# NSAPH-Projects/weather2alert

Hardware: AMD Instinct MI355X
Metric: env_steps_per_sec (higher is better)
Workload: dtype f32 tables, fp64 logit accumulation, f32 sigmoid/reward

## Files before the change

weather2alert_amd/csrc/w2a_step64.hip.h:

```cpp
#ifndef W2A_STEP64_HIP_H
#define W2A_STEP64_HIP_H

#ifndef W2A_S64_MIN_ENVS
#define W2A_S64_MIN_ENVS 131072
#endif
#define S64_ENVS 64
#define S64_WAVES (BLOCK / 64)
#define S64_PASS_ENVS 32
#define S64_ROUNDS 4

struct Day {
  uint32_t t, used, streak, hist, ndays, atb, actual, used2, hist2, st_bits, last;
  int32_t budget, act;
  bool done;
};
__device__ __forceinline__ Day derive_day(const u3 h, const u3 c, int32_t act) {
  Day d;
  d.st_bits = 0;
  if (act != 0 && act != 1) { d.st_bits |= W2A_ST_BAD_ACTION; act = 1; }
  d.act = act;
  d.last = D0_LAST(h.a);
  d.t = D0_T(h.a); d.used = D0_USED(h.a); d.streak = D0_STREAK(h.a);
  d.hist = D1_HIST(h.b); d.ndays = D1_NDAYS(h.b);
  d.budget = (int32_t)c.a;
  if (D1_FIN(h.b)) d.st_bits |= W2A_ST_STEP_AFTER_DONE;
  d.atb = ((int32_t)d.used == d.budget) ? 1u : 0u;
  d.actual = (act == 1 && d.atb) ? 0u : (uint32_t)act;
  d.used2 = d.used + d.actual;
  d.hist2 = ((d.hist << 1) | d.actual) & 0x3FFFu;
  d.done = (d.t + 1 >= d.ndays);
  return d;
}
__device__ __forceinline__ float4 runtime_fields(const Day &d, bool fix_lag = false) {
  return make_float4((d.t > 0) ? (float)(fix_lag ? d.last : d.actual) : 0.0f, (float)d.streak,
                     (float)(d.budget - (int32_t)d.used2), (float)__popc(d.hist2));
}
__device__ __forceinline__ void set_comp4(float4 &x, int idx, float v) {
  if (idx == 0) x.x = v;
  if (idx == 1) x.y = v;
  if (idx == 2) x.z = v;
  if (idx == 3) x.w = v;
}

template <bool FIXES>
struct S64WaveT {
  uint2 desc[S64_ENVS];
  float4 rt[S64_ENVS];
  float4 rt2[FIXES ? S64_ENVS : 1];
  float2 z[S64_ENVS];
  float tile[S64_PASS_ENVS * ROWF];
};

#ifndef W2A_S64_SC1
#define W2A_S64_SC1 0
#endif
#ifndef W2A_S64_SKIP_EFF
#define W2A_S64_SKIP_EFF 1
#endif
#ifndef W2A_S64_NT_STATE
#define W2A_S64_NT_STATE 0
#endif
typedef uint32_t v3u __attribute__((ext_vector_type(3)));
__device__ __forceinline__ void st16_sc1(void *p, v4f v) {
  asm volatile("global_store_dwordx4 %0, %1, off sc1" ::"v"(p), "v"(v) : "memory");
}
__device__ __forceinline__ void st12_sc1(void *p, v3u v) {
  asm volatile("global_store_dwordx3 %0, %1, off sc1" ::"v"(p), "v"(v) : "memory");
}
typedef uint32_t v2u __attribute__((ext_vector_type(2)));
__device__ __forceinline__ void st8_sc1(void *p, v2u v) {
  asm volatile("global_store_dwordx2 %0, %1, off sc1" ::"v"(p), "v"(v) : "memory");
}
__device__ __forceinline__ void st4_sc1(void *p, uint32_t v) {
  asm volatile("global_store_dword %0, %1, off sc1" ::"v"(p), "v"(v) : "memory");
}
__device__ __forceinline__ void st1_sc1(void *p, uint32_t v) {
  asm volatile("global_store_byte %0, %1, off sc1" ::"v"(p), "v"(v) : "memory");
}

#ifndef W2A_S64_MIN_WAVES
#define W2A_S64_MIN_WAVES 4
#endif
#ifndef W2A_S64_PRIO
#define W2A_S64_PRIO 3
#endif
#ifndef W2A_S64_TILES
#define W2A_S64_TILES 1
#endif
#ifndef W2A_S64_SERPENTINE
#define W2A_S64_SERPENTINE 1
#endif
__device__ __forceinline__ uint32_t logical_block_rev(uint32_t b, uint32_t per_xcd) {
#if W2A_XCD_SWIZZLE
  return (b & 7u) * per_xcd + (per_xcd - 1u - (b >> 3));
#else
  return 8u * per_xcd - 1u - b;
#endif
}
template <bool WRITE_OBS, bool REWARD_GIVEN, bool PACKED, bool AUTORESET = false, bool FIXES = false>
__device__ __forceinline__ void s64_tile(const StepArgs &a, S64WaveT<FIXES> &sw, const int lane, const int64_t wave_env0,
                                         const bool valid, const uint32_t e, const u3 h, const u3 c, const int32_t act,
                                         const int4 so) {
  const Day d = derive_day(h, c, act);
  const uint32_t t = d.t, used2 = d.used2, hist2 = d.hist2, streak = d.streak, ndays = d.ndays;
  const uint32_t actual = d.actual, atb = d.atb, st_bits = d.st_bits;
  const int32_t budget = d.budget;
  const bool done = d.done;
  const bool restart_in = AUTORESET && a.next_step && D1_FIN(h.b);
  const uint32_t fx = FIXES ? a.tb.fixes : 0u;
  const bool fix_obs = FIXES && WRITE_OBS && (fx & W2A_FIX_OBS);
  uint32_t need_eff = actual;
  if (a.tb.gate_bits && actual)
    need_eff = (a.tb.gate_bits[t * (uint32_t)a.tb.gate_words + (c.b >> 5)] >> (c.b & 31u)) & 1u;
  {
    const uint32_t day_row = t * (uint32_t)(a.tb.S_w * a.tb.Y) + c.b;
    const uint32_t wrow = W_COL(c.c) * (uint32_t)a.tb.n_samples + W_SAMPLE(c.c);
    sw.desc[lane] = make_uint2((day_row * (ROWF / 4)) | ((fix_obs && !done) ? 0x80000000u : 0u),
                               (wrow * (2 * ROWF / 4)) | (need_eff << 31));
    sw.rt[lane] = runtime_fields(d, (fx & W2A_FIX_LAG) != 0u);
    if (fix_obs)
      sw.rt2[FIXES ? lane : 0] = make_float4((float)actual, (float)(actual ? streak + 1 : 0), (float)(budget - (int32_t)used2),
                                 (float)__popc(hist2));
  }
  __builtin_amdgcn_fence(__ATOMIC_RELEASE, "wavefront");
  __builtin_amdgcn_wave_barrier();
  __builtin_amdgcn_fence(__ATOMIC_ACQUIRE, "wavefront");

  const int p = lane & 7;
  const int g = lane >> 3;
  const int n_obs = a.tb.n_obs;
  const bool write_me = valid && (!done || fix_obs) && !restart_in;
  const uint32_t next_day = (uint32_t)(a.tb.S_w * a.tb.Y) * (ROWF / 4);
#pragma unroll 1
  for (int pass = 0; pass < S64_ENVS / S64_PASS_ENVS; ++pass) {
    if (REWARD_GIVEN && !WRITE_OBS) break;
    if (wave_env0 + pass * S64_PASS_ENVS >= a.n) break;
    float4 x[S64_ROUNDS], wb[S64_ROUNDS], we[S64_ROUNDS], xo[FIXES ? S64_ROUNDS : 1];
    bool need[S64_ROUNDS], nxt[S64_ROUNDS];
#pragma unroll
    for (int r = 0; r < S64_ROUNDS; ++r) {
      uint2 ds = sw.desc[pass * S64_PASS_ENVS + r * 8 + g];
      need[r] = (ds.y >> 31) != 0u;
      nxt[r] = FIXES && (ds.x >> 31) != 0u;
      if (FIXES) ds.x &= 0x7FFFFFFFu;
      const uint32_t wq = ds.y & 0x7FFFFFFFu;
      x[r] = a.tb.X[ds.x + p];
      if (fix_obs) xo[r] = a.tb.X[ds.x + (nxt[r] ? next_day : 0u) + p];
      wb[r] = we[r] = make_float4(0.f, 0.f, 0.f, 0.f);
      if (!REWARD_GIVEN) {
        wb[r] = a.tb.W[wq + p];
        we[r] = a.tb.W[wq + (need[r] ? ROWF / 4 : 0) + p];
      }
    }
#if W2A_S64_PRIO
    __builtin_amdgcn_s_setprio(W2A_S64_PRIO);
#endif
#pragma unroll
    for (int r = 0; r < S64_ROUNDS; ++r) {
      const int j = pass * S64_PASS_ENVS + r * 8 + g;
      if (p == RT_QUAD) x[r] = sw.rt[j];
      if (FIXES && (fx & W2A_FIX_ALERTS_2WKS) && a.tb.slot_hist2w >= 0) {
        const float a2w = sw.rt[j].w;
        if (p == (a.tb.slot_hist2w >> 2)) set_comp4(x[r], a.tb.slot_hist2w & 3, a2w);
        if (fix_obs && p == (a.tb.slot_hist2w >> 2)) set_comp4(xo[r], a.tb.slot_hist2w & 3, a2w);
      }
      if (fix_obs && p == RT_QUAD) xo[r] = nxt[r] ? sw.rt2[FIXES ? j : 0] : sw.rt[j];
      if (!REWARD_GIVEN) {
      const double x0 = (double)x[r].x, x1 = (double)x[r].y, x2 = (double)x[r].z, x3 = (double)x[r].w;
      double zb = x0 * (double)wb[r].x;
      zb = fma(x1, (double)wb[r].y, zb);
      zb = fma(x2, (double)wb[r].z, zb);
      zb = fma(x3, (double)wb[r].w, zb);
      zb += dpp_f64<0xB1>(zb);
      zb += dpp_f64<0x4E>(zb);
      zb += dpp_f64<0x141>(zb);
      double ze = 0.0;
#if W2A_S64_SKIP_EFF
      if (__any(need[r]))
#endif
      {
        ze = x0 * (double)we[r].x;
        ze = fma(x1, (double)we[r].y, ze);
        ze = fma(x2, (double)we[r].z, ze);
        ze = fma(x3, (double)we[r].w, ze);
        if (p == GATE_QUAD && !(x[r].z > 0.5f)) ze = -__builtin_inf();
        ze += dpp_f64<0xB1>(ze);
        ze += dpp_f64<0x4E>(ze);
        ze += dpp_f64<0x141>(ze);
      }
      if (p == 0) sw.z[j] = make_float2((float)zb, (float)ze);
      }
      if (WRITE_OBS) {
        const int base = (r * 8 + g) * n_obs;
        const int trash = S64_PASS_ENVS * n_obs + (lane & 31);
        const float4 ov = fix_obs ? xo[FIXES ? r : 0] : x[r];
        sw.tile[so.x >= 0 ? base + so.x : trash] = ov.x;
        sw.tile[so.y >= 0 ? base + so.y : trash] = ov.y;
        sw.tile[so.z >= 0 ? base + so.z : trash] = ov.z;
        sw.tile[so.w >= 0 ? base + so.w : trash] = ov.w;
      }
    }
    if (WRITE_OBS) {
      __builtin_amdgcn_fence(__ATOMIC_RELEASE, "wavefront");
      __builtin_amdgcn_wave_barrier();
      __builtin_amdgcn_fence(__ATOMIC_ACQUIRE, "wavefront");
      const int64_t env0 = wave_env0 + pass * S64_PASS_ENVS;
      float *dst = reinterpret_cast<float *>(a.obs) + env0 * n_obs;
      const unsigned long long wm_all = __ballot(write_me);
      const uint32_t wm = (uint32_t)(wm_all >> (pass * S64_PASS_ENVS));
      const bool full = env0 + S64_PASS_ENVS <= a.n;
      if (full && wm == 0xFFFFFFFFu) {
        const int chunks = (S64_PASS_ENVS * n_obs) >> 2;
#pragma unroll
        for (int c0 = 0; c0 < (S64_PASS_ENVS * ROWF) / 4; c0 += 64) {
          const int ch = c0 + lane;
          if (ch < chunks) {
            const v4f v = reinterpret_cast<const v4f *>(sw.tile)[ch];
#if W2A_S64_SC1 & 1
            st16_sc1(reinterpret_cast<v4f *>(dst) + ch, v);
#elif W2A_NT_OBS
            __builtin_nontemporal_store(v, reinterpret_cast<v4f *>(dst) + ch);
#else
            reinterpret_cast<v4f *>(dst)[ch] = v;
#endif
          }
        }
      } else if (wm != 0u) {
        const int total = S64_PASS_ENVS * n_obs;
        for (int i = lane; i < total; i += 64) {
          const int jj = i / n_obs;
          if ((wm >> jj) & 1u) dst[i] = sw.tile[i];
        }
      }
      __builtin_amdgcn_fence(__ATOMIC_RELEASE, "wavefront");
      __builtin_amdgcn_wave_barrier();
      __builtin_amdgcn_fence(__ATOMIC_ACQUIRE, "wavefront");
    }
  }
  if (!WRITE_OBS) {
    __builtin_amdgcn_fence(__ATOMIC_RELEASE, "wavefront");
    __builtin_amdgcn_wave_barrier();
    __builtin_amdgcn_fence(__ATOMIC_ACQUIRE, "wavefront");
  }

#if W2A_S64_PRIO
  __builtin_amdgcn_s_setprio(0);
#endif
  if (AUTORESET && valid && restart_in) {
    a.reward[e] = 0.0f;
    a.done[e] = 0;
  } else if (valid && a.skip_finished && D1_FIN(h.b)) {
    a.reward[e] = 0.0f;
    a.done[e] = 1;
  } else if (valid) {
  float r;
  if (REWARD_GIVEN) {
    r = a.reward[e];
  } else {
    const float2 z = sw.z[lane];
    const float base = sigmoid_f32(z.x);
    const float eff = need_eff ? sigmoid_f32(z.y) : 0.0f;
    r = -(1000.0f / 152.0f) * base * (1.0f - eff);
    if (FIXES && (fx & W2A_FIX_PENALTY) && d.act == 1 && atb) r = -1.0f;
  }
  const uint32_t t2 = done ? t : t + 1;
  const uint32_t streak2 = done ? streak : (actual ? streak + 1 : 0);
  const float ret = __uint_as_float(h.c) + r;
  u3 h2;
  h2.a = pack_d0(t2, used2, streak2, actual, atb);
  h2.b = pack_d1(hist2, ndays, done ? 1u : 0u);
  h2.c = __float_as_uint(ret);
#if W2A_S64_SC1 & 2
  if (PACKED) st8_sc1(&a.st.pk_hot[e], v2u{pk_pack_hot(used2, streak2, hist2, done ? 1u : 0u), h2.c});
  else st12_sc1(&a.st.hot3[e], v3u{h2.a, h2.b, h2.c});
  if (!REWARD_GIVEN) st4_sc1(&a.reward[e], __float_as_uint(r));
  st1_sc1(&a.done[e], done ? 1u : 0u);
#else
  if (PACKED) a.st.pk_hot[e] = make_uint2(pk_pack_hot(used2, streak2, hist2, done ? 1u : 0u), h2.c);
  else a.st.hot3[e] = h2;
  if (!REWARD_GIVEN) a.reward[e] = r;
  a.done[e] = done ? 1 : 0;
#endif
  if (PACKED && lane == 0) a.st.pk_day[wave_env0 >> 6] = t2;
  if (done && a.last_return) a.last_return[e] = ret;
  if (st_bits) atomicOr(a.status, (int)st_bits);
  }
  if (AUTORESET) {
    const bool rs = valid && (a.next_step ? restart_in : done);
    const unsigned long long rs_mask = __ballot(rs);
    if (rs_mask) {
      uint2 ds = make_uint2(0xFFFFFFFFu, 0u);
      if (rs) {
        const uint4 cold = load_cold(a.st, e);
        const Episode ep = draw_episode(a.tb, a.rc, (uint64_t)(a.gid0 + e), cold.w + 1, (int32_t)cold.z);
        if (ep.bad) atomicOr(a.status, (int)W2A_ST_BAD_EPISODE);
        store_episode(a.st, e, make_uint4(ep.ep_row, ep.ep_w, (uint32_t)ep.sticky, cold.w + 1),
                      make_uint4(pack_d0(0, 0, 0, 0, 0), pack_d1(0, ep.ndays, 0), __float_as_uint(0.0f), (uint32_t)ep.budget));
        if (PACKED) {
          a.st.pk_hot[e] = make_uint2(pk_pack_hot(0u, 0u, 0u, 0u), __float_as_uint(0.0f));
          a.st.pk_c[e] = make_uint2(pk_budget16((uint32_t)ep.budget) | (W_COL(ep.ep_w) << 16),
                                    (ep.ep_row & 0x3FFFFFu) | (W_SAMPLE(ep.ep_w) << 22));
        }
        ds = make_uint2(ep.ep_row * (ROWF / 4), (uint32_t)ep.budget);
      }
      if (WRITE_OBS) {
        sw.desc[lane] = ds;
        __builtin_amdgcn_fence(__ATOMIC_RELEASE, "wavefront");
        __builtin_amdgcn_wave_barrier();
        __builtin_amdgcn_fence(__ATOMIC_ACQUIRE, "wavefront");
#pragma unroll 1
        for (int r = 0; r < S64_ENVS / 8; ++r) {
          if (!((rs_mask >> (r * 8)) & 0xFFull)) continue;
          const int j = r * 8 + g;
          const uint2 dj = sw.desc[j];
          if (dj.x != 0xFFFFFFFFu) {
            float4 v = a.tb.X[dj.x + p];
            if (p == RT_QUAD) v = make_float4(0.0f, 0.0f, (float)(int32_t)dj.y, 0.0f);
            if (FIXES && (fx & W2A_FIX_ALERTS_2WKS) && a.tb.slot_hist2w >= 0 && p == (a.tb.slot_hist2w >> 2))
              set_comp4(v, a.tb.slot_hist2w & 3, 0.0f);
            float *row = reinterpret_cast<float *>(a.obs) + (size_t)(wave_env0 + j) * n_obs;
            if (so.x >= 0) row[so.x] = v.x;
            if (so.y >= 0) row[so.y] = v.y;
            if (so.z >= 0) row[so.z] = v.z;
            if (so.w >= 0) row[so.w] = v.w;
          }
        }
      }
      if (PACKED && lane == 0) a.st.pk_day[wave_env0 >> 6] = 0u;
    }
  }
}

__device__ __forceinline__ void s64_load_packed(const StepArgs &a, uint32_t e, uint32_t day, u3 &h, u3 &c, int32_t &act) {
#if W2A_S64_NT_STATE & 4
  const v2u phv = __builtin_nontemporal_load(reinterpret_cast<const v2u *>(&a.st.pk_hot[e]));
  const v2u pcv = __builtin_nontemporal_load(reinterpret_cast<const v2u *>(&a.st.pk_c[e]));
  const uint2 ph = make_uint2(phv.x, phv.y), pc = make_uint2(pcv.x, pcv.y);
#else
  const uint2 ph = a.st.pk_hot[e];
  const uint2 pc = a.st.pk_c[e];
#endif
  h.a = pack_d0(day, PK_USED(ph.x), PK_STREAK(ph.x), PK_HIST(ph.x) & 1u, 0u);
  h.b = pack_d1(PK_HIST(ph.x), (uint32_t)a.uni_nd, PK_FIN(ph.x));
  h.c = ph.y;
  c.a = pc.x & 0xFFFFu;
  if (c.a == PK_BUDGET_ESCAPE) c.a = a.st.stepc[e].a;
  c.b = pc.y & 0x3FFFFFu;
  c.c = PACK_W(pc.x >> 16, pc.y >> 22);
  act = load_action(a, e);
}
__device__ __forceinline__ void s64_load_state(const StepArgs &a, uint32_t e, u3 &h, u3 &c, int32_t &act) {
#if W2A_S64_NT_STATE & 1
  const v3u hv = __builtin_nontemporal_load(reinterpret_cast<const v3u *>(&a.st.hot3[e]));
  h.a = hv.x; h.b = hv.y; h.c = hv.z;
#else
  h = a.st.hot3[e];
#endif
#if W2A_S64_NT_STATE & 2
  const v3u cv = __builtin_nontemporal_load(reinterpret_cast<const v3u *>(&a.st.stepc[e]));
  c.a = cv.x; c.b = cv.y; c.c = cv.z;
#else
  c = a.st.stepc[e];
#endif
  act = load_action(a, e);
}

template <bool WRITE_OBS, bool REWARD_GIVEN, bool PACKED = false, bool AUTORESET = false, bool FIXES = false>
__global__ __launch_bounds__(BLOCK, FIXES ? 3 : W2A_S64_MIN_WAVES) void k_step64(const StepArgs a) {
  __shared__ __attribute__((aligned(16))) S64WaveT<FIXES> s_w[S64_WAVES];
  const int tid = threadIdx.x;
  const int lane = tid & 63;
  const int wave = __builtin_amdgcn_readfirstlane(tid >> 6);
  S64WaveT<FIXES> &sw = s_w[wave];
  uint32_t lb = logical_block(blockIdx.x, gridDim.x >> 3);
  int wave_tile = wave;
#if W2A_S64_SERPENTINE
  if (a.walk_rev) {
    lb = logical_block_rev(blockIdx.x, gridDim.x >> 3);
    wave_tile = S64_WAVES - 1 - wave;
  }
#endif
  const int64_t wave_env0 = ((int64_t)lb * S64_WAVES + wave_tile) * (S64_ENVS * W2A_S64_TILES);
  if (wave_env0 >= a.n) return;
  uint32_t dayn = 0;
  if (PACKED) {
    dayn = a.st.pk_day[wave_env0 >> 6];
    if (dayn == W2A_PK_DAY_POISON) {
      if (lane == 0) atomicOr(a.status, (int)W2A_ST_STALE_GRAPH);
      return;
    }
  }
  u3 hn, cn;
  int32_t an;
  {
    const int64_t env = wave_env0 + lane;
    if (PACKED) s64_load_packed(a, (uint32_t)(env < a.n ? env : a.n - 1), dayn, hn, cn, an);
    else s64_load_state(a, (uint32_t)(env < a.n ? env : a.n - 1), hn, cn, an);
  }
  int4 so = make_int4(-1, -1, -1, -1);
  if (WRITE_OBS) so = reinterpret_cast<const int4 *>(a.slot_obs)[lane & 7];
#pragma unroll 1
  for (int i = 0; i < W2A_S64_TILES; ++i) {
    const int64_t env0 = wave_env0 + (int64_t)i * S64_ENVS;
    if (env0 >= a.n) break;
    const int64_t env = env0 + lane;
    const bool valid = env < a.n;
    const uint32_t e = (uint32_t)(valid ? env : (a.n - 1));
    const u3 h = hn, c = cn;
    const int32_t act = an;
    if (i + 1 < W2A_S64_TILES && env0 + S64_ENVS < a.n) {
      const int64_t en = env + S64_ENVS;
      if (PACKED) {
        dayn = a.st.pk_day[(env0 + S64_ENVS) >> 6];
        s64_load_packed(a, (uint32_t)(en < a.n ? en : a.n - 1), dayn == W2A_PK_DAY_POISON ? 0u : dayn, hn, cn, an);
      } else s64_load_state(a, (uint32_t)(en < a.n ? en : a.n - 1), hn, cn, an);
    }
    s64_tile<WRITE_OBS, REWARD_GIVEN, PACKED, AUTORESET, FIXES>(a, sw, lane, env0, valid, e, h, c, act, so);
    __builtin_amdgcn_fence(__ATOMIC_RELEASE, "wavefront");
    __builtin_amdgcn_wave_barrier();
    __builtin_amdgcn_fence(__ATOMIC_ACQUIRE, "wavefront");
  }
}

__global__ void k_pack_state(StateArrays st, int64_t n) {
  const int64_t i = (int64_t)blockIdx.x * blockDim.x + threadIdx.x;
  if (i >= n) return;
  const u3 h = st.hot3[i];
  const u3 c = st.stepc[i];
  st.pk_hot[i] = make_uint2(pk_pack_hot(D0_USED(h.a), D0_STREAK(h.a), D1_HIST(h.b), D1_FIN(h.b)), h.c);
  st.pk_c[i] = make_uint2(pk_budget16(c.a) | (W_COL(c.c) << 16), (c.b & 0x3FFFFFu) | (W_SAMPLE(c.c) << 22));
  if ((i & 63) == 0) st.pk_day[i >> 6] = D0_T(h.a);
}
__global__ void k_unpack_state(StateArrays st, int64_t n, int32_t n_days) {
  const int64_t i = (int64_t)blockIdx.x * blockDim.x + threadIdx.x;
  if (i >= n) return;
  const uint2 ph = st.pk_hot[i];
  const uint32_t t = st.pk_day[i >> 6];
  const uint32_t used = PK_USED(ph.x), hist = PK_HIST(ph.x), fin = PK_FIN(ph.x), last = hist & 1u;
  const uint32_t atb = ((t > 0 || fin) && (int32_t)(used - last) == (int32_t)st.stepc[i].a) ? 1u : 0u;
  u3 h;
  h.a = pack_d0(t, used, PK_STREAK(ph.x), last, atb);
  h.b = pack_d1(hist, (uint32_t)n_days, fin);
  h.c = ph.y;
  st.hot3[i] = h;
}
__global__ void k_poison_mirror(StateArrays st, int64_t n) {
  const int64_t i = (int64_t)blockIdx.x * blockDim.x + threadIdx.x;
  if (i < ((n + 63) >> 6)) st.pk_day[i] = W2A_PK_DAY_POISON;
}

#endif
```

Baseline: 30.95 billion.

## Software-pipeline table loads across both passes with a sliding slot window

Replaces the two-pass loop, where each pass issued all of its loads before computing, with a fully unrolled rolling window. Loads for the next rounds, including those of the second pass, are issued as soon as each slot is consumed. This lets X/W gathers for pass 1 overlap the compute and LDS flush of pass 0 instead of stalling at the pass boundary. The cost is higher register pressure and more code from full unrolling, and the old loop remains available behind the window macro.

```diff
diff --git a/weather2alert_amd/csrc/w2a_step64.hip.h b/weather2alert_amd/csrc/w2a_step64.hip.h
--- a/weather2alert_amd/csrc/w2a_step64.hip.h
+++ b/weather2alert_amd/csrc/w2a_step64.hip.h
@@ -86,6 +86,9 @@
 #endif
 #ifndef W2A_S64_TILES
 #define W2A_S64_TILES 1
+#endif
+#ifndef W2A_S64_WINDOW
+#define W2A_S64_WINDOW 4
 #endif
 #ifndef W2A_S64_SERPENTINE
 #define W2A_S64_SERPENTINE 1
@@ -131,59 +134,57 @@
   const int n_obs = a.tb.n_obs;
   const bool write_me = valid && (!done || fix_obs) && !restart_in;
   const uint32_t next_day = (uint32_t)(a.tb.S_w * a.tb.Y) * (ROWF / 4);
-#pragma unroll 1
-  for (int pass = 0; pass < S64_ENVS / S64_PASS_ENVS; ++pass) {
-    if (REWARD_GIVEN && !WRITE_OBS) break;
-    if (wave_env0 + pass * S64_PASS_ENVS >= a.n) break;
-    float4 x[S64_ROUNDS], wb[S64_ROUNDS], we[S64_ROUNDS], xo[FIXES ? S64_ROUNDS : 1];
-    bool need[S64_ROUNDS], nxt[S64_ROUNDS];
-#pragma unroll
-    for (int r = 0; r < S64_ROUNDS; ++r) {
-      uint2 ds = sw.desc[pass * S64_PASS_ENVS + r * 8 + g];
-      need[r] = (ds.y >> 31) != 0u;
-      nxt[r] = FIXES && (ds.x >> 31) != 0u;
+#if W2A_S64_WINDOW
+  constexpr int SLOTS = W2A_S64_WINDOW;
+#else
+  constexpr int SLOTS = S64_ROUNDS;
+#endif
+  struct Landing {
+    float4 x[SLOTS], wb[SLOTS], we[SLOTS], xo[FIXES ? SLOTS : 1];
+    bool need[SLOTS], nxt[SLOTS];
+  };
+  auto issue = [&](Landing &L, const int j0, const int r, const int s) __attribute__((always_inline)) {
+      uint2 ds = sw.desc[j0 + r * 8 + g];
+      L.need[s] = (ds.y >> 31) != 0u;
+      L.nxt[s] = FIXES && (ds.x >> 31) != 0u;
       if (FIXES) ds.x &= 0x7FFFFFFFu;
       const uint32_t wq = ds.y & 0x7FFFFFFFu;
-      x[r] = a.tb.X[ds.x + p];
-      if (fix_obs) xo[r] = a.tb.X[ds.x + (nxt[r] ? next_day : 0u) + p];
-      wb[r] = we[r] = make_float4(0.f, 0.f, 0.f, 0.f);
+      L.x[s] = a.tb.X[ds.x + p];
+      if (fix_obs) L.xo[FIXES ? s : 0] = a.tb.X[ds.x + (L.nxt[s] ? next_day : 0u) + p];
+      L.wb[s] = L.we[s] = make_float4(0.f, 0.f, 0.f, 0.f);
       if (!REWARD_GIVEN) {
-        wb[r] = a.tb.W[wq + p];
-        we[r] = a.tb.W[wq + (need[r] ? ROWF / 4 : 0) + p];
-      }
-    }
-#if W2A_S64_PRIO
-    __builtin_amdgcn_s_setprio(W2A_S64_PRIO);
-#endif
-#pragma unroll
-    for (int r = 0; r < S64_ROUNDS; ++r) {
-      const int j = pass * S64_PASS_ENVS + r * 8 + g;
-      if (p == RT_QUAD) x[r] = sw.rt[j];
+        L.wb[s] = a.tb.W[wq + p];
+        L.we[s] = a.tb.W[wq + (L.need[s] ? ROWF / 4 : 0) + p];
+      }
+  };
+  auto consume = [&](Landing &L, const int j0, const int r, const int s) __attribute__((always_inline)) {
+      const int j = j0 + r * 8 + g;
+      if (p == RT_QUAD) L.x[s] = sw.rt[j];
       if (FIXES && (fx & W2A_FIX_ALERTS_2WKS) && a.tb.slot_hist2w >= 0) {
         const float a2w = sw.rt[j].w;
-        if (p == (a.tb.slot_hist2w >> 2)) set_comp4(x[r], a.tb.slot_hist2w & 3, a2w);
-        if (fix_obs && p == (a.tb.slot_hist2w >> 2)) set_comp4(xo[r], a.tb.slot_hist2w & 3, a2w);
-      }
-      if (fix_obs && p == RT_QUAD) xo[r] = nxt[r] ? sw.rt2[FIXES ? j : 0] : sw.rt[j];
+        if (p == (a.tb.slot_hist2w >> 2)) set_comp4(L.x[s], a.tb.slot_hist2w & 3, a2w);
+        if (fix_obs && p == (a.tb.slot_hist2w >> 2)) set_comp4(L.xo[FIXES ? s : 0], a.tb.slot_hist2w & 3, a2w);
+      }
+      if (fix_obs && p == RT_QUAD) L.xo[FIXES ? s : 0] = L.nxt[s] ? sw.rt2[FIXES ? j : 0] : sw.rt[j];
       if (!REWARD_GIVEN) {
-      const double x0 = (double)x[r].x, x1 = (double)x[r].y, x2 = (double)x[r].z, x3 = (double)x[r].w;
-      double zb = x0 * (double)wb[r].x;
-      zb = fma(x1, (double)wb[r].y, zb);
-      zb = fma(x2, (double)wb[r].z, zb);
-      zb = fma(x3, (double)wb[r].w, zb);
+      const double x0 = (double)L.x[s].x, x1 = (double)L.x[s].y, x2 = (double)L.x[s].z, x3 = (double)L.x[s].w;
+      double zb = x0 * (double)L.wb[s].x;
+      zb = fma(x1, (double)L.wb[s].y, zb);
+      zb = fma(x2, (double)L.wb[s].z, zb);
+      zb = fma(x3, (double)L.wb[s].w, zb);
       zb += dpp_f64<0xB1>(zb);
       zb += dpp_f64<0x4E>(zb);
       zb += dpp_f64<0x141>(zb);
       double ze = 0.0;
 #if W2A_S64_SKIP_EFF
-      if (__any(need[r]))
+      if (__any(L.need[s]))
 #endif
       {
-        ze = x0 * (double)we[r].x;
-        ze = fma(x1, (double)we[r].y, ze);
-        ze = fma(x2, (double)we[r].z, ze);
-        ze = fma(x3, (double)we[r].w, ze);
-        if (p == GATE_QUAD && !(x[r].z > 0.5f)) ze = -__builtin_inf();
+        ze = x0 * (double)L.we[s].x;
+        ze = fma(x1, (double)L.we[s].y, ze);
+        ze = fma(x2, (double)L.we[s].z, ze);
+        ze = fma(x3, (double)L.we[s].w, ze);
+        if (p == GATE_QUAD && !(L.x[s].z > 0.5f)) ze = -__builtin_inf();
         ze += dpp_f64<0xB1>(ze);
         ze += dpp_f64<0x4E>(ze);
         ze += dpp_f64<0x141>(ze);
@@ -193,14 +194,14 @@
       if (WRITE_OBS) {
         const int base = (r * 8 + g) * n_obs;
         const int trash = S64_PASS_ENVS * n_obs + (lane & 31);
-        const float4 ov = fix_obs ? xo[FIXES ? r : 0] : x[r];
+        const float4 ov = fix_obs ? L.xo[FIXES ? s : 0] : L.x[s];
         sw.tile[so.x >= 0 ? base + so.x : trash] = ov.x;
         sw.tile[so.y >= 0 ? base + so.y : trash] = ov.y;
         sw.tile[so.z >= 0 ? base + so.z : trash] = ov.z;
         sw.tile[so.w >= 0 ? base + so.w : trash] = ov.w;
       }
-    }
-    if (WRITE_OBS) {
+  };
+  auto flush = [&](const int pass) __attribute__((always_inline)) {
       __builtin_amdgcn_fence(__ATOMIC_RELEASE, "wavefront");
       __builtin_amdgcn_wave_barrier();
       __builtin_amdgcn_fence(__ATOMIC_ACQUIRE, "wavefront");
@@ -235,8 +236,44 @@
       __builtin_amdgcn_fence(__ATOMIC_RELEASE, "wavefront");
       __builtin_amdgcn_wave_barrier();
       __builtin_amdgcn_fence(__ATOMIC_ACQUIRE, "wavefront");
+  };
+#if W2A_S64_WINDOW
+  static_assert(SLOTS >= S64_ROUNDS && SLOTS <= 2 * S64_ROUNDS, "W2A_S64_WINDOW: 0, or 4 .. 8 rounds");
+  auto rounds = [&](auto n_rounds) __attribute__((always_inline)) {
+    constexpr int NR = decltype(n_rounds)::value;
+    Landing L;
+#pragma unroll
+    for (int r = 0; r < SLOTS && r < NR; ++r) issue(L, (r / S64_ROUNDS) * S64_PASS_ENVS, r % S64_ROUNDS, r);
+#if W2A_S64_PRIO
+    __builtin_amdgcn_s_setprio(W2A_S64_PRIO);
+#endif
+#pragma unroll
+    for (int r = 0; r < NR; ++r) {
+      consume(L, (r / S64_ROUNDS) * S64_PASS_ENVS, r % S64_ROUNDS, r % SLOTS);
+      if (r + SLOTS < NR) issue(L, ((r + SLOTS) / S64_ROUNDS) * S64_PASS_ENVS, (r + SLOTS) % S64_ROUNDS, r % SLOTS);
+      if (WRITE_OBS && r % S64_ROUNDS == S64_ROUNDS - 1) flush(r / S64_ROUNDS);
     }
-  }
+  };
+  if (!(REWARD_GIVEN && !WRITE_OBS)) {
+    if (wave_env0 + S64_PASS_ENVS < a.n) rounds(std::integral_constant<int, 2 * S64_ROUNDS>());
+    else rounds(std::integral_constant<int, S64_ROUNDS>());
+  }
+#else
+#pragma unroll 1
+  for (int pass = 0; pass < S64_ENVS / S64_PASS_ENVS; ++pass) {
+    if (REWARD_GIVEN && !WRITE_OBS) break;
+    if (wave_env0 + pass * S64_PASS_ENVS >= a.n) break;
+    Landing L;
+#pragma unroll
+    for (int r = 0; r < S64_ROUNDS; ++r) issue(L, pass * S64_PASS_ENVS, r, r);
+#if W2A_S64_PRIO
+    __builtin_amdgcn_s_setprio(W2A_S64_PRIO);
+#endif
+#pragma unroll
+    for (int r = 0; r < S64_ROUNDS; ++r) consume(L, pass * S64_PASS_ENVS, r, r);
+    if (WRITE_OBS) flush(pass);
+  }
+#endif
   if (!WRITE_OBS) {
     __builtin_amdgcn_fence(__ATOMIC_RELEASE, "wavefront");
     __builtin_amdgcn_wave_barrier();
```

Result: no change. 31.17 billion (median of 6 runs) (+0.7%).
